# Perception4D/LidarSlam

Hardware: AMD Instinct MI355X
Metric: LiDAR frames/sec (AddFrame end-to-end), VLS-128 scan (higher is better)
Workload: dtype f32+f64; 1 GPU; VLS-128 synthetic spinning scan, street canyon, 5 m/s, EgoMotion=MOTION_EXTRAPOLATION_AND_REGISTRATION, Undistortion=REFINED, library defaults; points_per_frame=255802, sequences=1, parallelism=1 sequence per GPU x 1, frames_resident_in_hbm=False

## Files before the change

### lidarslam_amd/csrc/lsa_lm.hip

```cpp
#include <chrono>
#include <cmath>
#include "lsa_accum.h"
#include "lsa_device_math.h"
#include "lsa_sensor_terms.h"
#include "../../include/lsa_pmath.h"

using namespace lsa;

namespace
{

typedef unsigned long long u64;
#ifndef LSA_RECORD_PREFETCH
#define LSA_RECORD_PREFETCH 1
#endif
constexpr bool kRecordPrefetch = LSA_RECORD_PREFETCH != 0;

struct LmParams
{
  RecordSet set;
  double x0[6];
  int two_d;
  int max_iter;
  int min_matches;
  unsigned tag_base;
  int cslots;
  int give_up_block;
  const IcpLinkBlock* link;
  IcpLinkBlock* leave;
  int link_refine;
  int motion_from_args;
  posemath::ScanPoseClock clock;
  Rigid previous_world;
  double motion0[16];
  double* motion_dev;
  lsa_sensor_terms_t sensors;
  int sensors_on;
};

constexpr int kResPose = 0, kResInitial = 6, kResFinal = 7, kResSums = 8, kResSuccessful = 37, kResUnsuccessful = 38, kResIterations = 39,
              kResEvaluations = 40, kResSkipped = 41, kResCode = 42, kResMatches = 43, kResFailed = 44, kResCount = 45;
static_assert(kResCount <= kLmOut, "result does not fit the mailbox");

__device__ __forceinline__ constexpr int hidx(int a, int b) { return 7 + a * 6 - (a * (a - 1)) / 2 + (b - a); }
__device__ __forceinline__ constexpr int hsym(int a, int b) { return a <= b ? hidx(a, b) : hidx(b, a); }

struct LmState
{
  int cur_buf;
  double x[6], scale[6], diag[6];
  double radius, decrease_factor, x_norm, model_cost_change, delta_norm, initial_cost;
  int reuse_diagonal, consecutive_invalid, iter;
  int evaluations, successful, unsuccessful, iterations, code, skipped, matches;
};

struct Shared
{
  double wsum[kLmThreads / 64][kAccumVals];
  double part[kAccumVals][8];
  double sums[2][kAccumVals];
  double Hs[36], gs[6];
  double w[6];
  double rot[39];
  LmState lm;
  int failed;
  int stop;
  unsigned long long lap[6], tk;
  unsigned long long sub[4], st0;
};

__device__ __forceinline__ double uniform(double v)
{
  const long long b = __double_as_longlong(v);
  const int lo = __builtin_amdgcn_readfirstlane((int)(b & 0xffffffffll)), hi = __builtin_amdgcn_readfirstlane((int)(b >> 32));
  return __longlong_as_double(((long long)hi << 32) | (long long)(unsigned)lo);
}

__device__ __forceinline__ double lane_value(double v, int lane)
{
  const long long b = __double_as_longlong(v);
  const int lo = __shfl((int)(b & 0xffffffffll), lane), hi = __shfl((int)(b >> 32), lane);
  return __longlong_as_double(((long long)hi << 32) | (long long)(unsigned)lo);
}

__device__ __forceinline__ void lm_lap(Shared& sh, int slot)
{
  if (threadIdx.x == 0)
  {
    const unsigned long long now = wall_clock64();
    sh.lap[slot] += now - sh.tk;
    sh.tk = now;
  }
}

__device__ __noinline__ void lm_sensor_terms(const lsa_sensor_terms_t* terms, Shared& sh)
{
  sensor_terms_add(*terms, sh.w, sh.rot, sh.rot + 9, sh.rot + 18, sh.rot + 27, true, sh.sums[1 - sh.lm.cur_buf]);
}

__device__ __forceinline__ bool lm_evaluate(const LmParams& p, unsigned epoch, u64* __restrict__ xchg, Shared& sh, double* __restrict__ cache, bool trace)
{
  {
    RotConst c;
#pragma unroll
    for (int i = 0; i < 9; ++i) { c.R[i] = uniform(sh.rot[i]); c.dRx[i] = uniform(sh.rot[9 + i]); c.dRy[i] = uniform(sh.rot[18 + i]); c.dRz[i] = uniform(sh.rot[27 + i]); }
#pragma unroll
    for (int i = 0; i < 3; ++i) c.t[i] = uniform(sh.rot[36 + i]);
    double acc[kAccumVals];
#pragma unroll
    for (int v = 0; v < kAccumVals; ++v) acc[v] = 0.;
    const unsigned long long e0 = trace ? wall_clock64() : 0ull;
    accumulate_records_cached(p.set, c, blockIdx.x * blockDim.x + threadIdx.x, gridDim.x * blockDim.x, cache, p.cslots, p.cslots * kLmThreads, epoch == 1, kRecordPrefetch && p.cslots > 0 ? 1 : 0, acc);
    const unsigned long long e1 = trace ? wall_clock64() : 0ull;
    int slot;
    const double total = wave_reduce_accum(acc, slot);
    if (trace && threadIdx.x == 0) { sh.lap[4] += e1 - e0; }
    if ((threadIdx.x & 1) == 0 && slot < kAccumVals) sh.wsum[threadIdx.x >> 6][slot] = total;
  }
  if (threadIdx.x == 0) sh.failed = 0;
  __syncthreads();
  if (trace) lm_lap(sh, 0);
  const unsigned tag = p.tag_base + epoch;
  const int nb = gridDim.x;
  u64* slots = xchg + (size_t)(epoch & 1u) * kLmBlocksMax * kMailboxStride;
  if (threadIdx.x < 2 * kAccumVals)
  {
    const int v = threadIdx.x >> 1, half = threadIdx.x & 1;
    double r = sh.wsum[0][v];
#pragma unroll
    for (int w = 1; w < kLmThreads / 64; ++w) r += sh.wsum[w][v];
    const u64 bits = (u64)__double_as_longlong(r);
    const unsigned word = half ? (unsigned)(bits >> 32) : (unsigned)(bits & 0xffffffffull);
    __hip_atomic_store(slots + (size_t)blockIdx.x * kMailboxStride + threadIdx.x, ((u64)tag << 32) | word, __ATOMIC_RELAXED, __HIP_MEMORY_SCOPE_AGENT);
  }
  static_assert(kLmThreads / 64 == 8, "a wavefront per partial sum of the fold");
  bool failed = (int)blockIdx.x == p.give_up_block;
  {
    constexpr int kFoldBatch = 8;
    const int j = threadIdx.x >> 6, s = threadIdx.x & 63;
    const bool loads = s < 2 * kAccumVals;
    const u64* mine = slots + s;
    double sum = 0.;
    const unsigned long long t0 = wall_clock64();
    unsigned spins = 0;
    for (int b0 = j; b0 < nb; b0 += 8 * kFoldBatch)
    {
      u64 x[kFoldBatch];
#pragma unroll
      for (int k = 0; k < kFoldBatch; ++k) x[k] = 0ull;
      while (loads && !failed)
      {
#pragma unroll
        for (int k = 0; k < kFoldBatch; ++k)
          if (b0 + 8 * k < nb) x[k] = __hip_atomic_load(mine + (size_t)(b0 + 8 * k) * kMailboxStride, __ATOMIC_RELAXED, __HIP_MEMORY_SCOPE_AGENT);
        bool ok = true;
#pragma unroll
        for (int k = 0; k < kFoldBatch; ++k)
          if (b0 + 8 * k < nb && (unsigned)(x[k] >> 32) != tag) ok = false;
        if (ok) break;
        if ((++spins & 15u) == 0 && wall_clock64() - t0 > 2000000ull) { failed = true; break; }
        __builtin_amdgcn_s_sleep(2);
      }
#pragma unroll
      for (int k = 0; k < kFoldBatch; ++k)
      {
        const unsigned lo = (unsigned)(x[k] & 0xffffffffull);
        const unsigned hi = (unsigned)__builtin_amdgcn_update_dpp(0, (int)lo, 0xF5, 0xf, 0xf, false);
        if (b0 + 8 * k < nb) sum += __longlong_as_double((long long)(((u64)hi << 32) | lo));
      }
    }
    if (trace) lm_lap(sh, 1);
    if (loads && (s & 1) == 0) sh.part[s >> 1][j] = sum;
  }
  if (failed) atomicOr(&sh.failed, 1);
  __syncthreads();
  if (sh.failed) return false;
  if (threadIdx.x < kAccumVals)
  {
    double r = sh.part[threadIdx.x][0];
#pragma unroll
    for (int i = 1; i < 8; ++i) r += sh.part[threadIdx.x][i];
    sh.sums[1 - sh.lm.cur_buf][threadIdx.x] = r;
  }
  if (threadIdx.x < 64) asm volatile("s_waitcnt lgkmcnt(0)" ::: "memory");
  if (p.sensors_on && threadIdx.x == 0)
  {
    const char* args = (const char*)__builtin_amdgcn_kernarg_segment_ptr();
    const lsa_sensor_terms_t* terms = reinterpret_cast<const lsa_sensor_terms_t*>(args + offsetof(LmParams, sensors));
    lm_sensor_terms(terms, sh);
  }
  if (trace) lm_lap(sh, 2);
  return true;
}

enum LmCode
{
  kCodeNone = 0, kCodeNotEnoughMatches, kCodeGradient0, kCodeMaxIterations, kCodeGradient, kCodeMinRadius, kCodeInvalidSteps, kCodeParameterTolerance,
  kCodeFunctionTolerance
};

__device__ __forceinline__ void set_point(Shared& sh, const double w[6])
{
#pragma unroll
  for (int a = 0; a < 6; ++a) sh.w[a] = w[a];
}
__device__ __forceinline__ void finish_point(Shared& sh)
{
  asm volatile("s_waitcnt lgkmcnt(0)" ::: "memory");
  const int lane = threadIdx.x & 63;
  const double angle = sh.w[3 + (lane < 6 ? lane % 3 : 0)];
  const double v = lane < 3 ? lsa_cos(angle) : lsa_sin(angle);
  const double cx = lane_value(v, 0), cy = lane_value(v, 1), cz = lane_value(v, 2);
  const double sx = lane_value(v, 3), sy = lane_value(v, 4), sz = lane_value(v, 5);
  if (lane == 0)
  {
    double R[9], dRx[9], dRy[9], dRz[9];
    rotation_and_derivatives(cx, sx, cy, sy, cz, sz, R, dRx, dRy, dRz);
#pragma unroll
    for (int i = 0; i < 9; ++i) { sh.rot[i] = R[i]; sh.rot[9 + i] = dRx[i]; sh.rot[18 + i] = dRy[i]; sh.rot[27 + i] = dRz[i]; }
#pragma unroll
    for (int i = 0; i < 3; ++i) sh.rot[36 + i] = sh.w[i];
  }
}

template <int N> __device__ __forceinline__ constexpr int lm_act(int a) { return N == 6 ? a : (a == 2 ? 5 : a); }
template <int N>
__device__ __forceinline__ double lm_grad_max(const double* cur)
{
  double m = 0;
#pragma unroll
  for (int a = 0; a < N; ++a) { const double v = __builtin_fabs(cur[1 + lm_act<N>(a)]); m = m > v ? m : v; }
  return m;
}
template <int N>
__device__ bool lm_decide(const LmParams& p, Shared& sh, bool first)
{
  const double function_tolerance = 1e-6, gradient_tolerance = 1e-10, parameter_tolerance = 1e-8;
  const double min_relative_decrease = 1e-3, max_radius = 1e16;
  LmState& lm = sh.lm;
  const double* cur = sh.sums[lm.cur_buf];
  const double* tot = sh.sums[1 - lm.cur_buf];
  auto xnorm = [&]() {
    double s = 0;
#pragma unroll
    for (int a = 0; a < N; ++a) s += lm.x[lm_act<N>(a)] * lm.x[lm_act<N>(a)];
    return __builtin_sqrt(s);
  };

  if (first)
  {
    lm.matches = (int)tot[28];
    if (lm.matches < p.min_matches)
    {
      lm.skipped = 1;
      lm.code = kCodeNotEnoughMatches;
      return true;
    }
    lm.cur_buf ^= 1;
    cur = tot;
    lm.initial_cost = cur[0];
    lm.successful = 1;
#pragma unroll
    for (int a = 0; a < N; ++a) lm.scale[a] = 1.0 / (1.0 + __builtin_sqrt(cur[hidx(lm_act<N>(a), lm_act<N>(a))]));
    if (lm_grad_max<N>(cur) <= gradient_tolerance) { lm.code = kCodeGradient0; return true; }
    lm.x_norm = xnorm();
  }
  else
  {
    if (lm.delta_norm <= parameter_tolerance * (lm.x_norm + parameter_tolerance)) { lm.code = kCodeParameterTolerance; return true; }
    const double cost_change = cur[0] - tot[0];
    if (__builtin_fabs(cost_change) <= function_tolerance * cur[0]) { lm.code = kCodeFunctionTolerance; return true; }
    const double relative_decrease = cost_change / lm.model_cost_change;
    if (relative_decrease > min_relative_decrease)
    {
#pragma unroll
      for (int a = 0; a < 6; ++a) lm.x[a] = sh.w[a];
      lm.x_norm = xnorm();
      lm.cur_buf ^= 1;
      ++lm.successful;
      const double t = 2.0 * relative_decrease - 1.0;
      const double q = 1.0 - t * t * t;
      const double d = (1.0 / 3.0) < q ? q : (1.0 / 3.0);
      const double r = lm.radius / d;
      lm.radius = r < max_radius ? r : max_radius;
      lm.decrease_factor = 2.0;
      lm.reuse_diagonal = 0;
    }
    else
    {
      ++lm.unsuccessful;
      lm.radius /= lm.decrease_factor; lm.decrease_factor *= 2.0; lm.reuse_diagonal = 1;
    }
  }
  if (sh.st0) { const unsigned long long n = wall_clock64(); sh.sub[0] += n - sh.st0; sh.st0 = n; }
  return false;
}
template <int N>
__device__ __forceinline__ void lm_scale_system(Shared& sh)
{
  const int l = threadIdx.x & 63;
  const LmState& lm = sh.lm;
  const double* cur = sh.sums[lm.cur_buf];
  if (l < N * N)
  {
    const int a = l / N, b = l - a * N;
    const int fa = lm_act<N>(a), fb = lm_act<N>(b);
    const int lo = fa <= fb ? fa : fb, hi = fa <= fb ? fb : fa;
    sh.Hs[l] = cur[7 + lo * 6 - (lo * (lo - 1)) / 2 + (hi - lo)] * lm.scale[a] * lm.scale[b];
  }
  else if (l < N * N + N)
  {
    const int a = l - N * N;
    sh.gs[a] = cur[1 + lm_act<N>(a)] * lm.scale[a];
  }
}
template <int N>
__device__ bool lm_take_step(const LmParams& p, Shared& sh)
{
  const double gradient_tolerance = 1e-10, min_trust_region_radius = 1e-32;
  const double min_diagonal = 1e-6, max_diagonal = 1e32;
  const int max_consecutive_invalid = 5;
  LmState& lm = sh.lm;
  const double* cur = sh.sums[lm.cur_buf];
  double Hs[N * N], gs[N];
#pragma unroll
  for (int i = 0; i < N * N; ++i) Hs[i] = sh.Hs[i];
#pragma unroll
  for (int a = 0; a < N; ++a) gs[a] = sh.gs[a];
  while (true)
  {
    if (lm.iter >= p.max_iter) { lm.code = kCodeMaxIterations; return true; }
    if (lm_grad_max<N>(cur) <= gradient_tolerance) { lm.code = kCodeGradient; return true; }
    if (lm.radius < min_trust_region_radius) { lm.code = kCodeMinRadius; return true; }
    ++lm.iter;
    lm.iterations = lm.iter;
    if (!lm.reuse_diagonal)
    {
#pragma unroll
      for (int a = 0; a < N; ++a)
      {
        const double h = Hs[a * N + a];
        const double lo = h < min_diagonal ? min_diagonal : h;
        lm.diag[a] = max_diagonal < lo ? max_diagonal : lo;
      }
    }
    double M[N * N], y[N], step[N];
#pragma unroll
    for (int i = 0; i < N * N; ++i) M[i] = Hs[i];
#pragma unroll
    for (int a = 0; a < N; ++a) M[a * N + a] += lm.diag[a] / lm.radius;
#pragma unroll
    for (int a = 0; a < N; ++a) y[a] = 0.;
    if (sh.st0) { const unsigned long long n = wall_clock64(); sh.sub[1] += n - sh.st0; sh.st0 = n; }
    bool ok = solve_spd<N>(M, gs, y);
    if (sh.st0) { const unsigned long long n = wall_clock64(); sh.sub[2] += n - sh.st0; sh.st0 = n; }
    lm.reuse_diagonal = 1;
    double model_cost_change = 0;
    if (ok)
    {
#pragma unroll
      for (int a = 0; a < N; ++a) step[a] = -y[a];
      double sg = 0, sHs = 0;
#pragma unroll
      for (int a = 0; a < N; ++a)
      {
        sg += step[a] * gs[a];
        double t = 0;
#pragma unroll
        for (int b = 0; b < N; ++b) t += Hs[a * N + b] * step[b];
        sHs += step[a] * t;
      }
      model_cost_change = -sg - 0.5 * sHs;
      if (model_cost_change < 0.0) ok = false;
    }
    if (!ok)
    {
      ++lm.unsuccessful;
      if (++lm.consecutive_invalid >= max_consecutive_invalid) { lm.code = kCodeInvalidSteps; return true; }
      lm.radius /= lm.decrease_factor; lm.decrease_factor *= 2.0; lm.reuse_diagonal = 1;
      continue;
    }
    lm.consecutive_invalid = 0;
    lm.model_cost_change = model_cost_change;

    double cand[6], delta_norm = 0;
#pragma unroll
    for (int a = 0; a < 6; ++a) cand[a] = lm.x[a];
#pragma unroll
    for (int a = 0; a < N; ++a)
    {
      cand[lm_act<N>(a)] = lm.x[lm_act<N>(a)] + step[a] * lm.scale[a];
      const double e = lm.x[lm_act<N>(a)] - cand[lm_act<N>(a)];
      delta_norm += e * e;
    }
    lm.delta_norm = __builtin_sqrt(delta_norm);
    set_point(sh, cand);
    ++lm.evaluations;
    if (sh.st0) { const unsigned long long n = wall_clock64(); sh.sub[3] += n - sh.st0; sh.st0 = n; }
    return false;
  }
}
template <int N>
__device__ __forceinline__ void lm_step(const LmParams& p, Shared& sh, bool first)
{
  if (threadIdx.x == 0) sh.stop = lm_decide<N>(p, sh, first) ? 1 : 0;
  asm volatile("s_waitcnt lgkmcnt(0)" ::: "memory");
  if (sh.stop) return;
  lm_scale_system<N>(sh);
  asm volatile("s_waitcnt lgkmcnt(0)" ::: "memory");
  if (threadIdx.x == 0) sh.stop = lm_take_step<N>(p, sh) ? 1 : 0;
}

__device__ void leave_link(const LmParams& p, const LmState& lm, bool failed, int part)
{
  using namespace posemath;
  IcpLinkBlock* g = p.leave;
  const int lane = threadIdx.x & 63;
  const bool go = !failed && !lm.skipped && lm.successful != 1;
  if (!go)
  {
    if (lane == 0 && part == 0) g->go = 0ull;
    return;
  }
  if (part == 1 && !p.link_refine) return;
  const double half = lm.x[3 + (lane < 6 ? lane % 3 : 0)] * 0.5;
  const double v = lane < 3 ? lsa_cos(half) : lsa_sin(half);
  const double cx = lane_value(v, 0), cy = lane_value(v, 1), cz = lane_value(v, 2);
  const double sx = lane_value(v, 3), sy = lane_value(v, 4), sz = lane_value(v, 5);
  double x[6];
#pragma unroll
  for (int a = 0; a < 6; ++a) x[a] = lm.x[a];
  const Pose T = FromXYZRPYTrig(x, cx, sx, cy, sy, cz, sz);
  if (part == 0)
  {
    if (lane != 0) return;
    double x0[6];
    ToXYZRPY(T, x0);
    g->in.pose = ToRigid(T);
#pragma unroll
    for (int a = 0; a < 6; ++a) g->in.x0[a] = x0[a];
    g->go = 1ull;
    return;
  }
  WithinFrameMotion m;
  double mv[16];
#pragma unroll
  for (int i = 0; i < 16; ++i) mv[i] = p.motion0[i];
  if (!p.motion_from_args)
  {
#pragma unroll
    for (int i = 0; i < 16; ++i) mv[i] = p.motion_dev[i];
  }
  m.Time0 = mv[0]; m.Time1 = mv[1];
  m.Rot0 = {mv[2], mv[3], mv[4], mv[5]};
  m.Rot1 = {mv[6], mv[7], mv[8], mv[9]};
#pragma unroll
  for (int i = 0; i < 3; ++i) { m.Trans0[i] = mv[10 + i]; m.Trans1[i] = mv[13 + i]; }
  const Pose previous = FromRigid(p.previous_world);
  const Pose mine = InterpolateScanPose(p.clock, previous, T, lane == 1 ? m.Time1 : m.Time0);
  Pose worldToBaseEnd = Pose::Identity();
#pragma unroll
  for (int i = 0; i < 3; ++i)
#pragma unroll
    for (int j = 0; j < 4; ++j) worldToBaseEnd(i, j) = lane_value(mine(i, j), 1);
  if (lane != 0) return;
  Pose d0, d1;
  RefineUndistortionFrom(m, mine, worldToBaseEnd, T, d0, d1);
  g->in.ic = MakeInterpConst(d0, d1, m.Time0, m.Time1);
  double* o = p.motion_dev;
  o[0] = m.Time0; o[1] = m.Time1;
  o[2] = m.Rot0.w; o[3] = m.Rot0.x; o[4] = m.Rot0.y; o[5] = m.Rot0.z;
  o[6] = m.Rot1.w; o[7] = m.Rot1.x; o[8] = m.Rot1.y; o[9] = m.Rot1.z;
#pragma unroll
  for (int i = 0; i < 3; ++i) { o[10 + i] = m.Trans0[i]; o[13 + i] = m.Trans1[i]; }
}

__global__ __launch_bounds__(kLmThreads) void k_lm_solve(LmParams p, u64* __restrict__ xchg, u64* __restrict__ mailbox, unsigned out_tag, unsigned long long* trace)
{
  __shared__ Shared sh;
  extern __shared__ double lm_cache[];
  const bool tr = trace != nullptr && blockIdx.x == 0;
  RecordRegs pre;
  if (kRecordPrefetch && p.cslots > 0) record_load(p.set, blockIdx.x * blockDim.x + threadIdx.x, pre);
  if (p.link)
  {
    if (p.link->go != 1ull)
    {
      if (p.leave && blockIdx.x == 0 && threadIdx.x == 0) p.leave->go = 0ull;
      return;
    }
  }
  if (threadIdx.x == 0)
  {
    for (int i = 0; i < 6; ++i) sh.lap[i] = 0;
    for (int i = 0; i < 4; ++i) sh.sub[i] = 0;
    sh.st0 = 0;
    sh.tk = wall_clock64();
    sh.lap[5] = sh.tk;
    LmState& lm = sh.lm;
#pragma unroll
    for (int v = 0; v < kAccumVals; ++v) sh.sums[0][v] = 0.;
    lm.cur_buf = 0;
    double x0[6];
#pragma unroll
    for (int a = 0; a < 6; ++a) x0[a] = p.x0[a];
    if (p.link)
    {
#pragma unroll
      for (int a = 0; a < 6; ++a) x0[a] = p.link->in.x0[a];
    }
#pragma unroll
    for (int a = 0; a < 6; ++a) { lm.x[a] = x0[a]; lm.scale[a] = 1.; lm.diag[a] = 0.; }
    lm.radius = 1e4; lm.decrease_factor = 2.0; lm.x_norm = 0.; lm.model_cost_change = 0.; lm.delta_norm = 0.; lm.initial_cost = 0.;
    lm.reuse_diagonal = 0; lm.consecutive_invalid = 0; lm.iter = 0;
    lm.evaluations = 1; lm.successful = 0; lm.unsuccessful = 0; lm.iterations = 0; lm.code = kCodeNone; lm.skipped = 0; lm.matches = 0;
    set_point(sh, x0);
    sh.stop = 0;
  }
  if (threadIdx.x < 64) finish_point(sh);
  if (kRecordPrefetch && p.cslots > 0) record_stash(pre, lm_cache, p.cslots * kLmThreads, threadIdx.x);
  __syncthreads();
  bool failed = false;
  for (unsigned epoch = 1;; ++epoch)
  {
    if (!lm_evaluate(p, epoch, xchg, sh, lm_cache, tr)) { failed = true; break; }
    if (threadIdx.x < 64)
    {
      if (threadIdx.x == 0 && tr) sh.st0 = wall_clock64();
      if (p.two_d) lm_step<3>(p, sh, epoch == 1);
      else lm_step<6>(p, sh, epoch == 1);
      asm volatile("s_waitcnt lgkmcnt(0)" ::: "memory");
      if (!sh.stop) finish_point(sh);
    }
    __syncthreads();
    if (tr) lm_lap(sh, 3);
    if (sh.stop) break;
  }
  if (blockIdx.x != 0) return;
  if (tr && threadIdx.x == 0)
  {
    for (int i = 0; i < 4; ++i) trace[i] += sh.lap[i];
    trace[4] += (unsigned long long)sh.lm.evaluations;
    trace[5] += wall_clock64() - sh.lap[5];
    trace[6] += 1;
    trace[7] += sh.lap[4];
    for (int i = 0; i < 4; ++i) trace[8 + i] += sh.sub[i];
  }
  if (p.leave && threadIdx.x >= 64 && threadIdx.x < 192) leave_link(p, sh.lm, failed, (threadIdx.x >> 6) - 1);
  if (threadIdx.x < 2 * kResCount)
  {
    const LmState& lm = sh.lm;
    const int v = threadIdx.x >> 1, half = threadIdx.x & 1;
    double r = 0.;
    if (v < kResInitial) r = lm.x[v - kResPose];
    else if (v == kResInitial) r = lm.initial_cost;
    else if (v == kResFinal) r = sh.sums[lm.cur_buf][0];
    else if (v < kResSums + kAccumVals) r = sh.sums[lm.cur_buf][v - kResSums];
    else if (v == kResSuccessful) r = lm.successful;
    else if (v == kResUnsuccessful) r = lm.unsuccessful;
    else if (v == kResIterations) r = lm.iterations;
    else if (v == kResEvaluations) r = lm.evaluations;
    else if (v == kResSkipped) r = lm.skipped;
    else if (v == kResCode) r = lm.code;
    else if (v == kResMatches) r = lm.matches;
    else if (v == kResFailed) r = failed ? 1. : 0.;
    const u64 bits = (u64)__double_as_longlong(r);
    const unsigned word = half ? (unsigned)(bits >> 32) : (unsigned)(bits & 0xffffffffull);
    __hip_atomic_store(mailbox + threadIdx.x, ((u64)out_tag << 32) | word, __ATOMIC_RELAXED, __HIP_MEMORY_SCOPE_SYSTEM);
  }
}

const char* const kMessages[] = {"", "not enough matches", "gradient tolerance (iteration 0)", "max iterations", "gradient tolerance",
                                 "min trust region radius", "too many invalid steps", "parameter tolerance", "function tolerance"};

}

namespace lsa
{
std::atomic<int> g_live_contexts{0};
int lm_blocks_share()
{
  static const int cus = [] {
    hipDeviceProp_t prop;
    int dev = 0;
    if (hipGetDevice(&dev) != hipSuccess || hipGetDeviceProperties(&prop, dev) != hipSuccess) return 256;
    return std::max(prop.multiProcessorCount, 8);
  }();
  static const int queues = [] {
    const char* e = std::getenv("GPU_MAX_HW_QUEUES");
    const int q = e ? std::atoi(e) : 4;
    return std::max(q, 1);
  }();
  const int side_by_side = std::max(1, std::min(g_live_contexts.load(std::memory_order_relaxed), queues));
  return std::max(cus / side_by_side, 8);
}
int lm_cache_capacity()
{
  const size_t layer = (size_t)17 * kLmThreads * sizeof(double);
  size_t limit = 0, static_bytes = 0;
  {
    hipDeviceProp_t prop;
    int dev = 0;
    if (hipGetDevice(&dev) == hipSuccess && hipGetDeviceProperties(&prop, dev) == hipSuccess) limit = std::max(prop.sharedMemPerBlock, (size_t)prop.maxSharedMemoryPerMultiProcessor);
    hipFuncAttributes attr;
    if (hipFuncGetAttributes(&attr, reinterpret_cast<const void*>(k_lm_solve)) == hipSuccess) static_bytes = attr.sharedSizeBytes;
  }
  int slots = 0;
  for (int want = 3; want >= 1 && slots == 0; --want)
    if ((limit == 0 || static_bytes + want * layer <= limit) &&
        hipFuncSetAttribute(reinterpret_cast<const void*>(k_lm_solve), hipFuncAttributeMaxDynamicSharedMemorySize, (int)(want * layer)) == hipSuccess)
      slots = want;
  (void)hipGetLastError();
  return slots;
}
}

extern "C" {

static int solve_device_begin(lsa_ctx* ctx, unsigned type_mask, const double prior[6], int two_d_mode, int lm_max_iter, int min_matches, int leave_ticket, const lsa_icp_link_t* link)
{
  if (!ctx) return LSA_E_ARG;
  if (leave_ticket >= 0 && (leave_ticket >= kLinkRing || !link || !ctx->link_dev || !ctx->link_saved[leave_ticket].used))
    return ctx->fail(LSA_E_ARG, "lsa_solve_device_begin_linked: no such link (lsa_icp_link)");
  if (!prior && ctx->link_current < 0) return ctx->fail(LSA_E_ARG, "lsa_solve_device_begin: no start point and no link to wait behind");
  if (!ctx->lm_mailbox) return ctx->fail(LSA_E_STATE, "lsa_solve_device: no coherent host memory for the result");
  LSA_HIP(ctx, hipSetDevice(ctx->device));
  LmParams p;
  int total = 0;
  for (int k = 0; k < 3; ++k)
  {
    MatchBuf& mb = ctx->match[k];
    const bool use = (type_mask >> k) & 1u && mb.valid && mb.k > 0;
    p.set.rec[k] = mb.rec; p.set.status[k] = mb.status; p.set.cap[k] = mb.cap;
    p.set.count[k] = use ? mb.k : 0;
    p.set.sat2[k] = mb.sat * mb.sat;
    total += p.set.count[k];
  }
  for (int a = 0; a < 6; ++a) p.x0[a] = prior ? prior[a] : 0.;
  p.give_up_block = ctx->debug_lm_give_up_block;
  ctx->debug_lm_give_up_block = -1;
  p.link = prior ? nullptr : reinterpret_cast<const IcpLinkBlock*>(ctx->link_dev + (size_t)ctx->link_current * kLinkWords);
  p.leave = nullptr;
  p.link_refine = 0;
  p.motion_from_args = 0;
  p.motion_dev = ctx->motion_dev;
  std::memset(&p.clock, 0, sizeof(p.clock));
  std::memset(&p.previous_world, 0, sizeof(p.previous_world));
  std::memset(p.motion0, 0, sizeof(p.motion0));
  if (leave_ticket >= 0)
  {
    p.leave = reinterpret_cast<IcpLinkBlock*>(ctx->link_dev + (size_t)leave_ticket * kLinkWords);
    p.link_refine = link->refine_undistortion ? 1 : 0;
    p.motion_from_args = link->first ? 1 : 0;
    p.clock.have_log = link->have_log ? 1 : 0;
    p.clock.prev_time = link->prev_time;
    p.clock.cur_time = link->cur_time;
    p.clock.max_ratio = link->max_extrapolation_ratio;
    row_major_to_rt(link->previous_world, p.previous_world.R, p.previous_world.t);
    std::memcpy(p.motion0, link->motion, sizeof(p.motion0));
  }
  p.sensors = ctx->sensor_terms;
  p.sensors_on = (ctx->sensor_terms.wheel || ctx->sensor_terms.gravity) ? 1 : 0;
  p.two_d = two_d_mode ? 1 : 0;
  p.max_iter = lm_max_iter < 0 ? 0 : lm_max_iter;
  p.min_matches = min_matches;
  p.tag_base = ctx->lm_tag;
  ctx->lm_tag += (unsigned)p.max_iter + 4u;
  const unsigned out_tag = (unsigned)(++ctx->lm_seq);
  const int nb = std::min(std::max((total + ctx->lm_records - 1) / ctx->lm_records, 1), std::min(std::min(ctx->lm_blocks, kLmBlocksMax), lm_blocks_share()));
  const int per_thread = (total + nb * kLmThreads - 1) / (nb * kLmThreads);
  const size_t slot_bytes = (size_t)17 * kLmThreads * sizeof(double);
  p.cslots = std::min(per_thread, std::max(ctx->lm_cache_slots, 0));
  ctx->lm_shape[0] = nb; ctx->lm_shape[1] = per_thread; ctx->lm_shape[2] = p.cslots; ctx->lm_shape[3] = total;
  {
    ProfScope ps(ctx, "lm_solve", 0.);
    hipLaunchKernelGGL(k_lm_solve, dim3(nb), dim3(kLmThreads), p.cslots * slot_bytes, ctx->stream, p, ctx->lm_xchg, ctx->lm_mailbox + (size_t)(out_tag % kLmMailRing) * 2 * kLmOut, out_tag,
                       ctx->route_stats && ctx->trace_dev ? reinterpret_cast<unsigned long long*>(ctx->trace_dev) + (size_t)8192 * 12 : nullptr);
  }
  ctx->lm_pending.push_back(out_tag);
  ctx->lm_pending_wait.push_back(prior ? -1 : ctx->link_current);
  if (leave_ticket >= 0) ctx->link_current = leave_ticket;
  if (lsa_icp_trace_on()) std::fprintf(stderr, "[lm begin] tag %u linked %d leaves %d sat2 %.6g %.6g counts %d %d\n", out_tag, prior ? 0 : 1, leave_ticket, p.set.sat2[0], p.set.sat2[1], p.set.count[0], p.set.count[1]);
  return LSA_OK;
}

int lsa_solve_device_begin(lsa_ctx* ctx, unsigned type_mask, const double prior[6], int two_d_mode, int lm_max_iter, int min_matches)
{
  return solve_device_begin(ctx, type_mask, prior, two_d_mode, lm_max_iter, min_matches, -1, nullptr);
}

int lsa_solve_device_begin_linked(lsa_ctx* ctx, unsigned type_mask, const double prior[6], int two_d_mode, int lm_max_iter, int min_matches, int leave_ticket, const lsa_icp_link_t* link)
{
  if (ctx && (int)ctx->lm_pending.size() >= kLmMailRing - 1) return ctx->fail(LSA_E_STATE, "lsa_solve_device_begin_linked: too many solves in flight");
  return solve_device_begin(ctx, type_mask, prior, two_d_mode, lm_max_iter, min_matches, leave_ticket, link);
}

int lsa_solve_device_drop(lsa_ctx* ctx)
{
  if (!ctx || ctx->lm_pending.empty()) return LSA_E_ARG;
  ctx->lm_pending.pop_back();
  ctx->lm_pending_wait.pop_back();
  return LSA_OK;
}

int lsa_solve_device_end(lsa_ctx* ctx, lsa_solve_result_t* out)
{
  if (!ctx || !out) return ctx ? ctx->fail(LSA_E_ARG, "lsa_solve_device_end: bad argument") : LSA_E_ARG;
  if (ctx->lm_pending.empty()) return ctx->fail(LSA_E_STATE, "lsa_solve_device_end: no solve in flight");
  const unsigned out_tag = ctx->lm_pending.front();
  ctx->lm_pending.pop_front();
  const int waited_behind = ctx->lm_pending_wait.front();
  ctx->lm_pending_wait.pop_front();
  if (lsa_icp_trace_on()) std::fprintf(stderr, "[lm end] waits for tag %u (%zu more in flight)\n", out_tag, ctx->lm_pending.size());
  double res[kResCount];
  const unsigned long long* box = ctx->lm_mailbox + (size_t)(out_tag % kLmMailRing) * 2 * kLmOut;
  {
    const auto t0 = std::chrono::steady_clock::now();
    unsigned spins = 0;
    for (int v = 0; v < kResCount; ++v)
    {
      unsigned long long g[2];
      for (int h = 0; h < 2; ++h)
        while (((g[h] = __atomic_load_n(box + 2 * v + h, __ATOMIC_RELAXED)) >> 32) != out_tag)
        {
          if ((++spins & 0x3ff) == 0 && std::chrono::steady_clock::now() - t0 > std::chrono::milliseconds(2000))
          {
            (void)lsa_icp_abandon(ctx);
            LSA_HIP(ctx, hipStreamSynchronize(ctx->stream));
            return ctx->fail(LSA_E_STATE, "lsa_solve_device: no result from the device");
          }
#if defined(__x86_64__)
          __builtin_ia32_pause();
#endif
        }
      const unsigned long long bits = ((g[1] & 0xffffffffull) << 32) | (g[0] & 0xffffffffull);
      std::memcpy(&res[v], &bits, sizeof(double));
    }
  }
  if (lsa_icp_trace_on()) std::fprintf(stderr, "[lm end] tag %u: failed %g code %g evals %g matches %g\n", out_tag, res[kResFailed], res[kResCode], res[kResEvaluations], res[kResMatches]);
  if (res[kResFailed] != 0.)
  {
    (void)lsa_icp_abandon(ctx);
    LSA_HIP(ctx, hipStreamSynchronize(ctx->stream));
    ctx->lm_fallbacks++;
    return ctx->fail(LSA_E_STATE, "lsa_solve_device: a block waited too long for the others");
  }
  if (waited_behind >= 0 && waited_behind < kLinkRing) ctx->link_saved[waited_behind].used = false;
  std::memset(out, 0, sizeof(*out));
  for (int a = 0; a < 6; ++a) out->pose[a] = res[kResPose + a];
  out->initial_cost = res[kResInitial];
  out->final_cost = res[kResFinal];
  out->cost = res[kResSums];
  for (int a = 0; a < 6; ++a) out->g[a] = res[kResSums + 1 + a];
  {
    int h = kResSums + 7;
    for (int a = 0; a < 6; ++a)
      for (int b = a; b < 6; ++b) { out->H[a * 6 + b] = res[h]; out->H[b * 6 + a] = res[h]; ++h; }
  }
  out->num_successful_steps = (int)res[kResSuccessful];
  out->num_unsuccessful_steps = (int)res[kResUnsuccessful];
  out->num_iterations = (int)res[kResIterations];
  out->num_evaluations = (int)res[kResEvaluations];
  out->skipped = (int)res[kResSkipped];
  out->termination = (int)res[kResCode];
  out->num_matches = (int)res[kResMatches];
  out->message = kMessages[std::min(std::max(out->termination, 0), 8)];
  profile_add_bytes(ctx, "lm_solve", (double)out->num_evaluations * out->num_matches * 129);
  return LSA_OK;
}

int lsa_solve_device(lsa_ctx* ctx, unsigned type_mask, const double prior[6], int two_d_mode, int lm_max_iter, int min_matches, lsa_solve_result_t* out)
{
  if (!ctx || !prior || !out) return ctx ? ctx->fail(LSA_E_ARG, "lsa_solve_device: bad argument") : LSA_E_ARG;
  if (!ctx->lm_pending.empty()) return ctx->fail(LSA_E_STATE, "lsa_solve_device: another solve is in flight (lsa_solve_device_begin)");
  const int rc = lsa_solve_device_begin(ctx, type_mask, prior, two_d_mode, lm_max_iter, min_matches);
  if (rc) return rc;
  if (ctx->solve_hook)
  {
    void (*fn)(void*) = ctx->solve_hook;
    ctx->solve_hook = nullptr;
    fn(ctx->solve_hook_arg);
  }
  return lsa_solve_device_end(ctx, out);
}

int lsa_icp_link(lsa_ctx* ctx)
{
  if (!ctx) return LSA_E_ARG;
  if (!ctx->link_dev || !ctx->motion_dev) return ctx->fail(LSA_E_STATE, "lsa_icp_link: no device memory for the links");
  const unsigned seq = ctx->link_seq + 1;
  const int ticket = (int)(seq % kLinkRing);
  if (ctx->link_saved[ticket].used) return ctx->fail(LSA_E_STATE, "lsa_icp_link: too many iterations enqueued ahead");
  ctx->link_seq = seq;
  lsa_ctx::LinkSaved& sv = ctx->link_saved[ticket];
  sv = lsa_ctx::LinkSaved();
  sv.used = true;
  sv.seq = seq;
  return ticket;
}

int lsa_icp_link_expected(const double x[6], int skipped, int successful_steps, const lsa_icp_link_t* link, unsigned long long words[64], double motion_after[16])
{
  if (!x || !link || !words) return LSA_E_ARG;
  using namespace posemath;
  IcpLinkBlock g;
  std::memset(&g, 0, sizeof(g));
  std::memset(words, 0, kLinkWords * sizeof(unsigned long long));
  if (motion_after) std::memcpy(motion_after, link->motion, 16 * sizeof(double));
  if (skipped || successful_steps == 1) return LSA_OK;
  const Pose T = FromXYZRPY(x);
  ToXYZRPY(T, g.in.x0);
  g.in.pose = ToRigid(T);
  if (link->refine_undistortion)
  {
    WithinFrameMotion m;
    const double* mv = link->motion;
    m.Time0 = mv[0]; m.Time1 = mv[1];
    m.Rot0 = {mv[2], mv[3], mv[4], mv[5]};
    m.Rot1 = {mv[6], mv[7], mv[8], mv[9]};
    for (int i = 0; i < 3; ++i) { m.Trans0[i] = mv[10 + i]; m.Trans1[i] = mv[13 + i]; }
    ScanPoseClock clock;
    clock.have_log = link->have_log ? 1 : 0;
    clock.prev_time = link->prev_time;
    clock.cur_time = link->cur_time;
    clock.max_ratio = link->max_extrapolation_ratio;
    Pose previous, d0, d1;
    std::memcpy(previous.m, link->previous_world, sizeof(previous.m));
    previous = FromRigid(ToRigid(previous));
    RefineUndistortion(m, clock, previous, T, d0, d1);
    g.in.ic = MakeInterpConst(d0, d1, m.Time0, m.Time1);
    if (motion_after)
    {
      double* o = motion_after;
      o[0] = m.Time0; o[1] = m.Time1;
      o[2] = m.Rot0.w; o[3] = m.Rot0.x; o[4] = m.Rot0.y; o[5] = m.Rot0.z;
      o[6] = m.Rot1.w; o[7] = m.Rot1.x; o[8] = m.Rot1.y; o[9] = m.Rot1.z;
      for (int i = 0; i < 3; ++i) { o[10 + i] = m.Trans0[i]; o[13 + i] = m.Trans1[i]; }
    }
  }
  g.go = 1ull;
  std::memcpy(words, &g, sizeof(g));
  return LSA_OK;
}

int lsa_icp_link_peek(lsa_ctx* ctx, int ticket, unsigned long long words[64])
{
  if (!ctx || !words || ticket < 0 || ticket >= kLinkRing || !ctx->link_dev) return ctx ? ctx->fail(LSA_E_ARG, "lsa_icp_link_peek: bad argument") : LSA_E_ARG;
  LSA_HIP(ctx, hipSetDevice(ctx->device));
  LSA_HIP(ctx, hipStreamSynchronize(ctx->stream));
  LSA_HIP(ctx, hipMemcpy(words, ctx->link_dev + (size_t)ticket * kLinkWords, kLinkWords * sizeof(unsigned long long), hipMemcpyDeviceToHost));
  return LSA_OK;
}

int lsa_icp_cancel(lsa_ctx* ctx, int ticket)
{
  if (!ctx || ticket < 0 || ticket >= kLinkRing) return LSA_E_ARG;
  const lsa_ctx::LinkSaved sv = ctx->link_saved[ticket];
  if (!sv.used) return ctx->fail(LSA_E_ARG, "lsa_icp_cancel: no such link");
  ctx->link_saved[ticket].used = false;
  if (ctx->link_current == ticket) ctx->link_current = -1;
  for (int k = 0; k < 3; ++k)
    if ((sv.mask >> k) & 1u)
    {
      ctx->match[k].sat = sv.sat[k];
      ctx->match[k].k = sv.k[k];
      ctx->match[k].valid = sv.valid[k];
      ctx->hist_pos[k] = sv.hist_pos[k];
      ctx->hist_serial[k] = sv.hist_serial[k];
    }
  return LSA_OK;
}

int lsa_icp_abandon(lsa_ctx* ctx)
{
  if (!ctx) return LSA_E_ARG;
  while (true)
  {
    int youngest = -1;
    for (int t = 0; t < kLinkRing; ++t)
      if (ctx->link_saved[t].used && (youngest < 0 || (int)(ctx->link_saved[t].seq - ctx->link_saved[youngest].seq) > 0)) youngest = t;
    if (youngest < 0) break;
    if (lsa_icp_cancel(ctx, youngest) != LSA_OK) ctx->link_saved[youngest].used = false;
  }
  ctx->lm_pending.clear();
  ctx->lm_pending_wait.clear();
  ctx->link_current = -1;
  return LSA_OK;
}

int lsa_debug_set(lsa_ctx* ctx, const char* name, int value)
{
  if (!ctx || !name) return LSA_E_ARG;
  const std::string n(name);
  const lsa_ctx::ShapeKnobs& c = ctx->created_knobs;
  if (n == "lm_give_up_block") ctx->debug_lm_give_up_block = value;
  else if (n == "lm_blocks") ctx->lm_blocks = value < 0 ? c.lm_blocks : std::min(std::max(value, 1), kLmBlocksMax);
  else if (n == "lm_records") ctx->lm_records = value < 0 ? c.lm_records : std::min(std::max(value, 256), 4096);
  else if (n == "lm_cache") ctx->lm_cache_slots = value < 0 ? c.lm_cache_slots : std::min(value, ctx->lm_cache_capacity);
  else if (n == "accum_blocks") ctx->accum_blocks = value < 0 ? c.accum_blocks : std::min(std::max(value, 1), kAccumBlocksMax);
  else if (n == "mailbox_check") ctx->mailbox_check = value < 0 ? c.mailbox_check : value != 0;
  else if (n == "pcd_lds") ctx->pcd_lds = value < 0 ? -1 : (value != 0);
  else if (n == "kplog_chunk_kib") ctx->kplog_chunk_bytes = value < 0 ? ((size_t)32 << 20) : (size_t)std::max(value, 1) << 10;
  else if (n == "kplog_fail_alloc") ctx->debug_kplog_fail_alloc = value > 0 ? 1 : 0;
  else if (n == "place_max_blocks") ctx->place_max_blocks = value > 0 ? value : 0;
  else return ctx->fail(LSA_E_ARG, "lsa_debug_set: no such knob");
  return LSA_OK;
}

int lsa_solve_device_shape(const lsa_ctx* ctx, int out[4])
{
  if (!ctx || !out) return LSA_E_ARG;
  std::memcpy(out, ctx->lm_shape, sizeof(ctx->lm_shape));
  return LSA_OK;
}

int lsa_accumulate_shape(const lsa_ctx* ctx, int out[4])
{
  if (!ctx || !out) return LSA_E_ARG;
  std::memcpy(out, ctx->accum_shape, sizeof(ctx->accum_shape));
  return LSA_OK;
}

int lsa_solve_device_fallbacks(const lsa_ctx* ctx) { return ctx ? ctx->lm_fallbacks : 0; }

int lsa_set_sensor_terms(lsa_ctx* ctx, const lsa_sensor_terms_t* terms)
{
  if (!ctx) return LSA_E_ARG;
  if (terms) ctx->sensor_terms = *terms;
  else std::memset(&ctx->sensor_terms, 0, sizeof(ctx->sensor_terms));
  return LSA_OK;
}

int lsa_solve_device_interlude(lsa_ctx* ctx, void (*fn)(void*), void* arg)
{
  if (!ctx) return LSA_E_ARG;
  ctx->solve_hook = fn;
  ctx->solve_hook_arg = arg;
  return LSA_OK;
}

int lsa_solve_device_trace(lsa_ctx* ctx, unsigned long long out[12])
{
  if (!ctx || !out || !ctx->trace_dev) return LSA_E_ARG;
  if (hipStreamSynchronize(ctx->stream) != hipSuccess) return LSA_E_HIP;
  if (hipMemcpy(out, reinterpret_cast<unsigned long long*>(ctx->trace_dev) + (size_t)8192 * 12, 12 * sizeof(unsigned long long), hipMemcpyDeviceToHost) != hipSuccess) return LSA_E_HIP;
  return LSA_OK;
}

}
```

Before: 1429 frames/s.

## Spread LM trust-region step across wavefront lanes with register-resident Cholesky

Rewrites the per-iteration Levenberg-Marquardt decide/scale/solve step. It used to run serially on thread 0 with LDS round-trips between phases; it now runs wave-parallel, with each lane holding one Hessian row and doing a lane-broadcast Cholesky solve. State is kept in registers and written back to shared memory once, and the candidate pose goes straight into finish_point instead of through shared memory. It also swaps ds_bpermute shuffles for readlane broadcasts. This targets the serial latency of the solver in the iteration loop, at the cost of more intricate code and some risk of numerical or bookkeeping divergence from the original solver.

```diff
diff --git a/lidarslam_amd/csrc/lsa_lm.hip b/lidarslam_amd/csrc/lsa_lm.hip
--- a/lidarslam_amd/csrc/lsa_lm.hip
+++ b/lidarslam_amd/csrc/lsa_lm.hip
@@ -83,6 +83,13 @@
   return __longlong_as_double(((long long)hi << 32) | (long long)(unsigned)lo);
 }
 
+__device__ __forceinline__ double lane_bcast(double v, int src)
+{
+  const long long b = __double_as_longlong(v);
+  const int lo = __builtin_amdgcn_readlane((int)(b & 0xffffffffll), src), hi = __builtin_amdgcn_readlane((int)(b >> 32), src);
+  return __longlong_as_double(((long long)hi << 32) | (long long)(unsigned)lo);
+}
+
 __device__ __forceinline__ void lm_lap(Shared& sh, int slot)
 {
   if (threadIdx.x == 0)
@@ -199,19 +206,16 @@
   kCodeFunctionTolerance
 };
 
-__device__ __forceinline__ void set_point(Shared& sh, const double w[6])
-{
-#pragma unroll
-  for (int a = 0; a < 6; ++a) sh.w[a] = w[a];
-}
-__device__ __forceinline__ void finish_point(Shared& sh)
-{
-  asm volatile("s_waitcnt lgkmcnt(0)" ::: "memory");
-  const int lane = threadIdx.x & 63;
-  const double angle = sh.w[3 + (lane < 6 ? lane % 3 : 0)];
+__device__ __forceinline__ void finish_point(Shared& sh, double x, double y, double z, double rx, double ry, double rz)
+{
+  const double w[6] = {x, y, z, rx, ry, rz};
+  int lane = threadIdx.x & 63;
+  asm volatile("" : "+v"(lane));
+  const int k = lane < 6 ? lane % 3 : 0;
+  const double angle = k == 0 ? rx : (k == 1 ? ry : rz);
   const double v = lane < 3 ? lsa_cos(angle) : lsa_sin(angle);
-  const double cx = lane_value(v, 0), cy = lane_value(v, 1), cz = lane_value(v, 2);
-  const double sx = lane_value(v, 3), sy = lane_value(v, 4), sz = lane_value(v, 5);
+  const double cx = lane_bcast(v, 0), cy = lane_bcast(v, 1), cz = lane_bcast(v, 2);
+  const double sx = lane_bcast(v, 3), sy = lane_bcast(v, 4), sz = lane_bcast(v, 5);
   if (lane == 0)
   {
     double R[9], dRx[9], dRy[9], dRz[9];
@@ -219,196 +223,271 @@
 #pragma unroll
     for (int i = 0; i < 9; ++i) { sh.rot[i] = R[i]; sh.rot[9 + i] = dRx[i]; sh.rot[18 + i] = dRy[i]; sh.rot[27 + i] = dRz[i]; }
 #pragma unroll
-    for (int i = 0; i < 3; ++i) sh.rot[36 + i] = sh.w[i];
+    for (int i = 0; i < 3; ++i) sh.rot[36 + i] = w[i];
+#pragma unroll
+    for (int a = 0; a < 6; ++a) sh.w[a] = w[a];
   }
 }
 
 template <int N> __device__ __forceinline__ constexpr int lm_act(int a) { return N == 6 ? a : (a == 2 ? 5 : a); }
 template <int N>
-__device__ __forceinline__ double lm_grad_max(const double* cur)
+__device__ __forceinline__ double lm_grad_max(const double g[N])
 {
   double m = 0;
 #pragma unroll
-  for (int a = 0; a < N; ++a) { const double v = __builtin_fabs(cur[1 + lm_act<N>(a)]); m = m > v ? m : v; }
+  for (int a = 0; a < N; ++a) { const double v = __builtin_fabs(g[a]); m = m > v ? m : v; }
   return m;
 }
 template <int N>
-__device__ bool lm_decide(const LmParams& p, Shared& sh, bool first)
+__device__ __forceinline__ double lm_x_norm(const double x[6])
+{
+  double s = 0;
+#pragma unroll
+  for (int a = 0; a < N; ++a) s += x[lm_act<N>(a)] * x[lm_act<N>(a)];
+  return __builtin_sqrt(s);
+}
+template <int N>
+__device__ __forceinline__ bool lm_step(const LmParams& p, Shared& sh, bool first, double cand[6])
 {
   const double function_tolerance = 1e-6, gradient_tolerance = 1e-10, parameter_tolerance = 1e-8;
-  const double min_relative_decrease = 1e-3, max_radius = 1e16;
+  const double min_relative_decrease = 1e-3, max_radius = 1e16, min_trust_region_radius = 1e-32;
+  const double min_diagonal = 1e-6, max_diagonal = 1e32;
+  const int max_consecutive_invalid = 5;
+  int lane = threadIdx.x & 63;
+  asm volatile("" : "+v"(lane));
+  const bool l0 = lane == 0;
+  const int row = lane < N ? lane : 0;
+  const int fr = N == 6 ? row : (row == 2 ? 5 : row);
   LmState& lm = sh.lm;
-  const double* cur = sh.sums[lm.cur_buf];
-  const double* tot = sh.sums[1 - lm.cur_buf];
-  auto xnorm = [&]() {
-    double s = 0;
-#pragma unroll
-    for (int a = 0; a < N; ++a) s += lm.x[lm_act<N>(a)] * lm.x[lm_act<N>(a)];
-    return __builtin_sqrt(s);
+  unsigned long long t0 = sh.st0;
+  auto stamp = [&](int part) {
+    if (t0 && l0) { const unsigned long long n = wall_clock64(); sh.sub[part] += n - t0; t0 = n; }
   };
 
+  int cur_buf = lm.cur_buf;
+  const double* tot = sh.sums[1 - cur_buf];
+  const double* old = sh.sums[cur_buf];
+  const double tot_cost = tot[0], old_cost = old[0], tot_count = tot[28];
+  double tot_g[N], old_g[N], tot_row[N], kept_row[N], kept_gs[N], scale[N], x_old[6], x_w[6];
+#pragma unroll
+  for (int a = 0; a < N; ++a)
+  {
+    const int fb = lm_act<N>(a);
+    const int lo = fr <= fb ? fr : fb, hi = fr <= fb ? fb : fr;
+    tot_g[a] = tot[1 + fb];
+    old_g[a] = old[1 + fb];
+    tot_row[a] = tot[7 + lo * 6 - (lo * (lo - 1)) / 2 + (hi - lo)];
+    kept_row[a] = sh.Hs[row * N + a];
+    kept_gs[a] = sh.gs[a];
+    scale[a] = lm.scale[a];
+  }
+#pragma unroll
+  for (int a = 0; a < 6; ++a) { x_old[a] = lm.x[a]; x_w[a] = sh.w[a]; }
+  double scale_row = lm.scale[row], diag_row = lm.diag[row];
+  double radius = lm.radius, decrease_factor = lm.decrease_factor, x_norm = lm.x_norm, model_cost_change = lm.model_cost_change, delta_norm = lm.delta_norm;
+  int reuse_diagonal = lm.reuse_diagonal, consecutive_invalid = lm.consecutive_invalid, iter = lm.iter;
+  int successful = lm.successful, unsuccessful = lm.unsuccessful, evaluations = lm.evaluations;
+  double tot_diag = tot_row[0];
+#pragma unroll
+  for (int b = 1; b < N; ++b)
+    if (row == b) tot_diag = tot_row[b];
+
+  bool use_tot;
   if (first)
   {
-    lm.matches = (int)tot[28];
-    if (lm.matches < p.min_matches)
-    {
-      lm.skipped = 1;
-      lm.code = kCodeNotEnoughMatches;
+    const int matches = (int)tot_count;
+    if (l0) lm.matches = matches;
+    if (matches < p.min_matches)
+    {
+      if (l0) { lm.skipped = 1; lm.code = kCodeNotEnoughMatches; sh.stop = 1; }
       return true;
     }
-    lm.cur_buf ^= 1;
-    cur = tot;
-    lm.initial_cost = cur[0];
-    lm.successful = 1;
-#pragma unroll
-    for (int a = 0; a < N; ++a) lm.scale[a] = 1.0 / (1.0 + __builtin_sqrt(cur[hidx(lm_act<N>(a), lm_act<N>(a))]));
-    if (lm_grad_max<N>(cur) <= gradient_tolerance) { lm.code = kCodeGradient0; return true; }
-    lm.x_norm = xnorm();
+    use_tot = true;
+    successful = 1;
+    scale_row = 1.0 / (1.0 + __builtin_sqrt(tot_diag));
+#pragma unroll
+    for (int a = 0; a < N; ++a) scale[a] = lane_bcast(scale_row, a);
+    if (lane < N) lm.scale[lane] = scale_row;
+    if (l0) { lm.initial_cost = tot_cost; lm.cur_buf = cur_buf ^ 1; lm.successful = 1; }
+    if (lm_grad_max<N>(tot_g) <= gradient_tolerance)
+    {
+      if (l0) { lm.code = kCodeGradient0; sh.stop = 1; }
+      return true;
+    }
+    x_norm = lm_x_norm<N>(x_old);
   }
   else
   {
-    if (lm.delta_norm <= parameter_tolerance * (lm.x_norm + parameter_tolerance)) { lm.code = kCodeParameterTolerance; return true; }
-    const double cost_change = cur[0] - tot[0];
-    if (__builtin_fabs(cost_change) <= function_tolerance * cur[0]) { lm.code = kCodeFunctionTolerance; return true; }
-    const double relative_decrease = cost_change / lm.model_cost_change;
-    if (relative_decrease > min_relative_decrease)
-    {
-#pragma unroll
-      for (int a = 0; a < 6; ++a) lm.x[a] = sh.w[a];
-      lm.x_norm = xnorm();
-      lm.cur_buf ^= 1;
-      ++lm.successful;
+    if (delta_norm <= parameter_tolerance * (x_norm + parameter_tolerance))
+    {
+      if (l0) { lm.code = kCodeParameterTolerance; sh.stop = 1; }
+      return true;
+    }
+    const double cost_change = old_cost - tot_cost;
+    if (__builtin_fabs(cost_change) <= function_tolerance * old_cost)
+    {
+      if (l0) { lm.code = kCodeFunctionTolerance; sh.stop = 1; }
+      return true;
+    }
+    const double relative_decrease = cost_change / model_cost_change;
+    use_tot = relative_decrease > min_relative_decrease;
+    if (use_tot)
+    {
+      x_norm = lm_x_norm<N>(x_w);
+      ++successful;
       const double t = 2.0 * relative_decrease - 1.0;
       const double q = 1.0 - t * t * t;
       const double d = (1.0 / 3.0) < q ? q : (1.0 / 3.0);
-      const double r = lm.radius / d;
-      lm.radius = r < max_radius ? r : max_radius;
-      lm.decrease_factor = 2.0;
-      lm.reuse_diagonal = 0;
+      const double r = radius / d;
+      radius = r < max_radius ? r : max_radius;
+      decrease_factor = 2.0;
+      reuse_diagonal = 0;
     }
     else
     {
-      ++lm.unsuccessful;
-      lm.radius /= lm.decrease_factor; lm.decrease_factor *= 2.0; lm.reuse_diagonal = 1;
-    }
-  }
-  if (sh.st0) { const unsigned long long n = wall_clock64(); sh.sub[0] += n - sh.st0; sh.st0 = n; }
-  return false;
-}
-template <int N>
-__device__ __forceinline__ void lm_scale_system(Shared& sh)
-{
-  const int l = threadIdx.x & 63;
-  const LmState& lm = sh.lm;
-  const double* cur = sh.sums[lm.cur_buf];
-  if (l < N * N)
-  {
-    const int a = l / N, b = l - a * N;
-    const int fa = lm_act<N>(a), fb = lm_act<N>(b);
-    const int lo = fa <= fb ? fa : fb, hi = fa <= fb ? fb : fa;
-    sh.Hs[l] = cur[7 + lo * 6 - (lo * (lo - 1)) / 2 + (hi - lo)] * lm.scale[a] * lm.scale[b];
-  }
-  else if (l < N * N + N)
-  {
-    const int a = l - N * N;
-    sh.gs[a] = cur[1 + lm_act<N>(a)] * lm.scale[a];
-  }
-}
-template <int N>
-__device__ bool lm_take_step(const LmParams& p, Shared& sh)
-{
-  const double gradient_tolerance = 1e-10, min_trust_region_radius = 1e-32;
-  const double min_diagonal = 1e-6, max_diagonal = 1e32;
-  const int max_consecutive_invalid = 5;
-  LmState& lm = sh.lm;
-  const double* cur = sh.sums[lm.cur_buf];
-  double Hs[N * N], gs[N];
-#pragma unroll
-  for (int i = 0; i < N * N; ++i) Hs[i] = sh.Hs[i];
-#pragma unroll
-  for (int a = 0; a < N; ++a) gs[a] = sh.gs[a];
+      ++unsuccessful;
+      radius /= decrease_factor; decrease_factor *= 2.0; reuse_diagonal = 1;
+    }
+  }
+  if (use_tot) cur_buf ^= 1;
+  stamp(0);
+
+  double x[6], g[N], Hrow[N], gs[N];
+#pragma unroll
+  for (int a = 0; a < 6; ++a) x[a] = use_tot ? x_w[a] : x_old[a];
+#pragma unroll
+  for (int a = 0; a < N; ++a)
+  {
+    g[a] = use_tot ? tot_g[a] : old_g[a];
+    const double h = tot_row[a] * scale_row * scale[a];
+    const double gsa = tot_g[a] * scale[a];
+    Hrow[a] = use_tot ? h : kept_row[a];
+    gs[a] = use_tot ? gsa : kept_gs[a];
+  }
+  if (use_tot)
+  {
+    if (lane < N)
+    {
+#pragma unroll
+      for (int a = 0; a < N; ++a) sh.Hs[lane * N + a] = Hrow[a];
+    }
+    if (l0)
+    {
+#pragma unroll
+      for (int a = 0; a < N; ++a) sh.gs[a] = gs[a];
+    }
+  }
+  const double grad_max = lm_grad_max<N>(g);
+  double Hdiag = Hrow[0];
+#pragma unroll
+  for (int b = 1; b < N; ++b)
+    if (row == b) Hdiag = Hrow[b];
+
+  int code = kCodeNone;
   while (true)
   {
-    if (lm.iter >= p.max_iter) { lm.code = kCodeMaxIterations; return true; }
-    if (lm_grad_max<N>(cur) <= gradient_tolerance) { lm.code = kCodeGradient; return true; }
-    if (lm.radius < min_trust_region_radius) { lm.code = kCodeMinRadius; return true; }
-    ++lm.iter;
-    lm.iterations = lm.iter;
-    if (!lm.reuse_diagonal)
-    {
-#pragma unroll
-      for (int a = 0; a < N; ++a)
-      {
-        const double h = Hs[a * N + a];
-        const double lo = h < min_diagonal ? min_diagonal : h;
-        lm.diag[a] = max_diagonal < lo ? max_diagonal : lo;
-      }
-    }
-    double M[N * N], y[N], step[N];
-#pragma unroll
-    for (int i = 0; i < N * N; ++i) M[i] = Hs[i];
-#pragma unroll
-    for (int a = 0; a < N; ++a) M[a * N + a] += lm.diag[a] / lm.radius;
-#pragma unroll
-    for (int a = 0; a < N; ++a) y[a] = 0.;
-    if (sh.st0) { const unsigned long long n = wall_clock64(); sh.sub[1] += n - sh.st0; sh.st0 = n; }
-    bool ok = solve_spd<N>(M, gs, y);
-    if (sh.st0) { const unsigned long long n = wall_clock64(); sh.sub[2] += n - sh.st0; sh.st0 = n; }
-    lm.reuse_diagonal = 1;
-    double model_cost_change = 0;
-    if (ok)
-    {
-#pragma unroll
-      for (int a = 0; a < N; ++a) step[a] = -y[a];
-      double sg = 0, sHs = 0;
-#pragma unroll
-      for (int a = 0; a < N; ++a)
-      {
-        sg += step[a] * gs[a];
-        double t = 0;
-#pragma unroll
-        for (int b = 0; b < N; ++b) t += Hs[a * N + b] * step[b];
-        sHs += step[a] * t;
-      }
-      model_cost_change = -sg - 0.5 * sHs;
-      if (model_cost_change < 0.0) ok = false;
-    }
-    if (!ok)
-    {
-      ++lm.unsuccessful;
-      if (++lm.consecutive_invalid >= max_consecutive_invalid) { lm.code = kCodeInvalidSteps; return true; }
-      lm.radius /= lm.decrease_factor; lm.decrease_factor *= 2.0; lm.reuse_diagonal = 1;
+    if (iter >= p.max_iter) { code = kCodeMaxIterations; break; }
+    if (grad_max <= gradient_tolerance) { code = kCodeGradient; break; }
+    if (radius < min_trust_region_radius) { code = kCodeMinRadius; break; }
+    ++iter;
+    if (!reuse_diagonal)
+    {
+      const double lo = Hdiag < min_diagonal ? min_diagonal : Hdiag;
+      diag_row = max_diagonal < lo ? max_diagonal : lo;
+    }
+    double s[N];
+    const double damped = Hdiag + diag_row / radius;
+#pragma unroll
+    for (int j = 0; j < N; ++j) s[j] = row == j ? damped : Hrow[j];
+    if (lane == N)
+    {
+#pragma unroll
+      for (int j = 0; j < N; ++j) s[j] = gs[j];
+    }
+    stamp(1);
+    bool ok = true;
+    double rinv[N], Lu[N + 1][N];
+#pragma unroll
+    for (int j = 0; j < N; ++j)
+    {
+      const double d = lane_bcast(s[j], j);
+      if (!(d > 0.0) || !isfinite(d)) ok = false;
+      rinv[j] = 1.0 / __builtin_sqrt(d);
+      const double lij = s[j] * rinv[j];
+#pragma unroll
+      for (int jj = j + 1; jj <= N; ++jj) Lu[jj][j] = lane_bcast(lij, jj);
+#pragma unroll
+      for (int jj = j + 1; jj < N; ++jj) s[jj] -= lij * Lu[jj][j];
+    }
+    double y[N];
+#pragma unroll
+    for (int i = N - 1; i >= 0; --i)
+    {
+      double t = Lu[N][i];
+#pragma unroll
+      for (int k = i + 1; k < N; ++k) t -= Lu[k][i] * y[k];
+      y[i] = t * rinv[i];
+    }
+#pragma unroll
+    for (int i = 0; i < N; ++i)
+      if (!isfinite(y[i])) ok = false;
+    stamp(2);
+    reuse_diagonal = 1;
+    double step[N], t_row = 0, sg = 0, sHs = 0;
+#pragma unroll
+    for (int a = 0; a < N; ++a) step[a] = -y[a];
+#pragma unroll
+    for (int b = 0; b < N; ++b) t_row += Hrow[b] * step[b];
+#pragma unroll
+    for (int a = 0; a < N; ++a)
+    {
+      sg += step[a] * gs[a];
+      sHs += step[a] * lane_bcast(t_row, a);
+    }
+    const double change = -sg - 0.5 * sHs;
+    if (!ok || change < 0.0)
+    {
+      ++unsuccessful;
+      if (++consecutive_invalid >= max_consecutive_invalid) { code = kCodeInvalidSteps; break; }
+      radius /= decrease_factor; decrease_factor *= 2.0;
       continue;
     }
-    lm.consecutive_invalid = 0;
-    lm.model_cost_change = model_cost_change;
-
-    double cand[6], delta_norm = 0;
-#pragma unroll
-    for (int a = 0; a < 6; ++a) cand[a] = lm.x[a];
+    consecutive_invalid = 0;
+    model_cost_change = change;
+    double dn = 0;
+#pragma unroll
+    for (int a = 0; a < 6; ++a) cand[a] = x[a];
 #pragma unroll
     for (int a = 0; a < N; ++a)
     {
-      cand[lm_act<N>(a)] = lm.x[lm_act<N>(a)] + step[a] * lm.scale[a];
-      const double e = lm.x[lm_act<N>(a)] - cand[lm_act<N>(a)];
-      delta_norm += e * e;
-    }
-    lm.delta_norm = __builtin_sqrt(delta_norm);
-    set_point(sh, cand);
-    ++lm.evaluations;
-    if (sh.st0) { const unsigned long long n = wall_clock64(); sh.sub[3] += n - sh.st0; sh.st0 = n; }
-    return false;
-  }
-}
-template <int N>
-__device__ __forceinline__ void lm_step(const LmParams& p, Shared& sh, bool first)
-{
-  if (threadIdx.x == 0) sh.stop = lm_decide<N>(p, sh, first) ? 1 : 0;
-  asm volatile("s_waitcnt lgkmcnt(0)" ::: "memory");
-  if (sh.stop) return;
-  lm_scale_system<N>(sh);
-  asm volatile("s_waitcnt lgkmcnt(0)" ::: "memory");
-  if (threadIdx.x == 0) sh.stop = lm_take_step<N>(p, sh) ? 1 : 0;
+      cand[lm_act<N>(a)] = x[lm_act<N>(a)] + step[a] * scale[a];
+      const double e = x[lm_act<N>(a)] - cand[lm_act<N>(a)];
+      dn += e * e;
+    }
+    delta_norm = __builtin_sqrt(dn);
+    ++evaluations;
+    break;
+  }
+
+  if (lane < N) lm.diag[lane] = diag_row;
+  if (l0)
+  {
+    if (use_tot && !first)
+    {
+#pragma unroll
+      for (int a = 0; a < 6; ++a) lm.x[a] = x[a];
+    }
+    lm.cur_buf = cur_buf;
+    lm.x_norm = x_norm; lm.radius = radius; lm.decrease_factor = decrease_factor;
+    lm.model_cost_change = model_cost_change; lm.delta_norm = delta_norm;
+    lm.reuse_diagonal = reuse_diagonal; lm.consecutive_invalid = consecutive_invalid;
+    lm.iter = iter; lm.iterations = iter;
+    lm.successful = successful; lm.unsuccessful = unsuccessful; lm.evaluations = evaluations;
+    lm.code = code;
+    sh.stop = code != kCodeNone ? 1 : 0;
+  }
+  stamp(3);
+  return code != kCodeNone;
 }
 
 __device__ void leave_link(const LmParams& p, const LmState& lm, bool failed, int part)
@@ -490,17 +569,8 @@
       return;
     }
   }
-  if (threadIdx.x == 0)
-  {
-    for (int i = 0; i < 6; ++i) sh.lap[i] = 0;
-    for (int i = 0; i < 4; ++i) sh.sub[i] = 0;
-    sh.st0 = 0;
-    sh.tk = wall_clock64();
-    sh.lap[5] = sh.tk;
-    LmState& lm = sh.lm;
-#pragma unroll
-    for (int v = 0; v < kAccumVals; ++v) sh.sums[0][v] = 0.;
-    lm.cur_buf = 0;
+  if (threadIdx.x < 64)
+  {
     double x0[6];
 #pragma unroll
     for (int a = 0; a < 6; ++a) x0[a] = p.x0[a];
@@ -509,15 +579,26 @@
 #pragma unroll
       for (int a = 0; a < 6; ++a) x0[a] = p.link->in.x0[a];
     }
-#pragma unroll
-    for (int a = 0; a < 6; ++a) { lm.x[a] = x0[a]; lm.scale[a] = 1.; lm.diag[a] = 0.; }
-    lm.radius = 1e4; lm.decrease_factor = 2.0; lm.x_norm = 0.; lm.model_cost_change = 0.; lm.delta_norm = 0.; lm.initial_cost = 0.;
-    lm.reuse_diagonal = 0; lm.consecutive_invalid = 0; lm.iter = 0;
-    lm.evaluations = 1; lm.successful = 0; lm.unsuccessful = 0; lm.iterations = 0; lm.code = kCodeNone; lm.skipped = 0; lm.matches = 0;
-    set_point(sh, x0);
-    sh.stop = 0;
-  }
-  if (threadIdx.x < 64) finish_point(sh);
+    if (threadIdx.x == 0)
+    {
+      for (int i = 0; i < 6; ++i) sh.lap[i] = 0;
+      for (int i = 0; i < 4; ++i) sh.sub[i] = 0;
+      sh.st0 = 0;
+      sh.tk = wall_clock64();
+      sh.lap[5] = sh.tk;
+      LmState& lm = sh.lm;
+#pragma unroll
+      for (int v = 0; v < kAccumVals; ++v) sh.sums[0][v] = 0.;
+      lm.cur_buf = 0;
+#pragma unroll
+      for (int a = 0; a < 6; ++a) { lm.x[a] = x0[a]; lm.scale[a] = 1.; lm.diag[a] = 0.; }
+      lm.radius = 1e4; lm.decrease_factor = 2.0; lm.x_norm = 0.; lm.model_cost_change = 0.; lm.delta_norm = 0.; lm.initial_cost = 0.;
+      lm.reuse_diagonal = 0; lm.consecutive_invalid = 0; lm.iter = 0;
+      lm.evaluations = 1; lm.successful = 0; lm.unsuccessful = 0; lm.iterations = 0; lm.code = kCodeNone; lm.skipped = 0; lm.matches = 0;
+      sh.stop = 0;
+    }
+    finish_point(sh, x0[0], x0[1], x0[2], x0[3], x0[4], x0[5]);
+  }
   if (kRecordPrefetch && p.cslots > 0) record_stash(pre, lm_cache, p.cslots * kLmThreads, threadIdx.x);
   __syncthreads();
   bool failed = false;
@@ -527,10 +608,9 @@
     if (threadIdx.x < 64)
     {
       if (threadIdx.x == 0 && tr) sh.st0 = wall_clock64();
-      if (p.two_d) lm_step<3>(p, sh, epoch == 1);
-      else lm_step<6>(p, sh, epoch == 1);
-      asm volatile("s_waitcnt lgkmcnt(0)" ::: "memory");
-      if (!sh.stop) finish_point(sh);
+      double cand[6];
+      const bool stop = p.two_d ? lm_step<3>(p, sh, epoch == 1, cand) : lm_step<6>(p, sh, epoch == 1, cand);
+      if (!stop) finish_point(sh, cand[0], cand[1], cand[2], cand[3], cand[4], cand[5]);
     }
     __syncthreads();
     if (tr) lm_lap(sh, 3);
```

Result: faster. 1454 frames/s (median of 6 runs) (+1.8%).
